# mikasenghaas/diloco-swarm

Measured on AMD Instinct MI355X. Metric: GB/s params reduced (device-resident), DiLoCo outer step @1/2/4/8 GPU, higher is better.
Workload: dtype f32; 1 GPU; DiLoCo outer step, t125 tree per rank, through the reference's calls (src/train.py:263-269) on get_outer_model's default (CPU) outer model, stepped on its HBM twin: one dl_delta_pack_sgd per step (delta + outer.grad + Nesterov SGD + copy to inner; no exchange at one replica, src/comm.py:118-119); tree=t125, placement=host (write_back lazy: HBM twin), params=124475904, tensors=148, wire=f32, buckets=2, exchange=none (one peer), parallelism=dp1

## Files before the change

### __graft_entry__.py

```python
import os
import subprocess
import sys

HERE = os.path.dirname(os.path.abspath(__file__))
PKG = os.path.join(HERE, "diloco-swarm_amd")
for _p in (PKG, HERE):
    if _p not in sys.path:
        sys.path.insert(0, _p)


def build() -> None:
    env = dict(os.environ)
    env.setdefault("PYTORCH_ROCM_ARCH", "gfx950")
    subprocess.run(["make", "-s", "-C", os.path.join(PKG, "csrc")], check=True, env=env)
    subprocess.run(["make", "-s", "-C", os.path.join(HERE, "oracle")], check=True, env=env)
    cabi = os.path.join(HERE, "tests", "cabi")
    subprocess.run(
        ["gcc", "-O2", "-std=c11", "-D__HIP_PLATFORM_AMD__", "-I/opt/rocm/include",
         os.path.join(cabi, "host_step.c"), "-o", os.path.join(cabi, "host_step"),
         "-L" + os.path.join(PKG, "lib"), "-ldiloco_hip", "-L" + os.path.join(HERE, "oracle"),
         "-loracle", "-L/opt/rocm/lib", "-lamdhip64",
         "-Wl,-rpath,$ORIGIN/../../diloco-swarm_amd/lib", "-Wl,-rpath,$ORIGIN/../../oracle",
         "-Wl,-rpath,/opt/rocm/lib"], check=True, env=env)
    import diloco_amd
    from diloco_amd import _lib

    _lib.load()


def smoke() -> None:
    import numpy as np
    import torch

    from diloco_amd import synth
    from diloco_amd.outer import OuterSync
    from diloco_amd.trees import get_tree
    from oracle import oracle

    dev = torch.device("cuda", 0)
    spec = get_tree("micro")
    shapes = [s for _, s in spec.params()]
    params = [t.view(s) for t, s in zip(synth.outer_tree_device(spec, dev), shapes)]
    eng = OuterSync(params, lr=0.7, momentum=0.9, nesterov=True, world_size=1, keep_wire=True)
    synth.inner_tree_device([p.view(-1) for p in params], 1, 0, out=[p.view(-1) for p in params])
    eng.step()
    torch.cuda.synchronize()
    got = np.concatenate([t.reshape(-1).cpu().numpy() for t in eng.unpacked(eng.theta)])
    inner = np.concatenate([p.reshape(-1).cpu().numpy() for p in params])
    wire = np.concatenate([t.reshape(-1).cpu().numpy() for t in eng.unpacked(eng.wire)])

    with np.load(os.path.join(HERE, "tests", "golden", "micro_n1.npz")) as g:
        ref_theta, ref_delta = g["theta_s1"], g["delta_s1_r0"]
    st = oracle.OuterState(synth.outer_tree(spec.numels(), spec.init_spec()))
    deltas, _ = st.step([synth.inner_tree(st.theta, 1, 0)])
    assert got.tobytes() == ref_theta.tobytes(), "HIP outer step != reference (micro, n=1)"
    assert got.tobytes() == np.concatenate(st.theta).tobytes(), "HIP outer step != oracle"
# ... 37 lines not shown
```

### diloco-swarm_amd/csrc/dl_abi.hip

```cpp
#include <cstdarg>
#include <cstdio>
#include <cstring>
#include <new>
#include <string>
#include <vector>

#include "dl_internal.h"

namespace {

thread_local std::string g_err;

int fail(int code, const char* fmt, ...) __attribute__((format(printf, 2, 3)));
int fail(int code, const char* fmt, ...) {
  char buf[512];
  va_list ap;
  va_start(ap, fmt);
  vsnprintf(buf, sizeof buf, fmt, ap);
  va_end(ap);
  g_err = buf;
  return code;
}

int hip_fail(hipError_t e, const char* where) {
// ... 39 lines not shown
}

struct dl_tree_s;
namespace {
int slot_begin(dl_tree_s* t, int32_t slot, hipStream_t s, const char* who);
int slot_end(dl_tree_s* t, int32_t slot, hipStream_t s, const char* who);
}

constexpr int kStageRing = 4;

struct dl_tree_s {
  int device = 0;
  int32_t nseg = 0;
  int64_t total = 0;
  std::vector<int64_t> numel, seg_off, bounds;
  std::vector<int32_t> bkt_chunk;
  std::vector<dl::Chunk> chunks;
  std::vector<int64_t> chunk_loff;
  dl::Chunk* d_chunks = nullptr;
  int64_t* d_loff = nullptr;
  void** d_caddr = nullptr;
  uint64_t* d_segptr = nullptr;
  uint64_t* h_stage = nullptr;
  hipEvent_t stage_ev[kStageRing] = {};
  bool stage_used[kStageRing] = {};
  int stage_next = 0;
  std::vector<uint8_t> bound;
  std::vector<uint8_t> slot_aligned;
  int32_t grid = 0;
  int32_t flags = DL_TUNE_AUTO;
  hipEvent_t slot_ev[DL_MAX_SLOTS] = {};
  hipStream_t slot_stream[DL_MAX_SLOTS] = {};
  bool slot_used[DL_MAX_SLOTS] = {};
};

namespace {
int slot_begin(dl_tree_s* t, int32_t slot, hipStream_t s, const char* who) {
  if (slot < 0) return DL_OK;
  if (t->slot_used[slot] && t->slot_stream[slot] != s)
    DL_HIP(hipStreamWaitEvent(s, t->slot_ev[slot], 0), who);
  return DL_OK;
}
int slot_end(dl_tree_s* t, int32_t slot, hipStream_t s, const char* who) {
  if (slot < 0) return DL_OK;
  DL_HIP(hipEventRecord(t->slot_ev[slot], s), who);
  t->slot_stream[slot] = s;
  t->slot_used[slot] = true;
  return DL_OK;
}
}

extern "C" {

DL_API const char* dl_last_error(void) { return g_err.c_str(); }
DL_API int dl_abi_version(void) { return DL_ABI_VERSION; }

DL_API int dl_plan_tables_ex(const int64_t* numel, int32_t n, int64_t cap_elems,
                             int32_t align_elems, int64_t bucket_align_elems, int64_t* seg_off,
                             int64_t* bkt_bounds, int32_t* n_bkt) {
  if (n < 0 || (n > 0 && !numel) || !seg_off || !bkt_bounds || !n_bkt)
    return fail(DL_E_ARG, "dl_plan_tables: null pointer or n < 0");
  if (align_elems <= 0) return fail(DL_E_ARG, "dl_plan_tables: align_elems must be > 0");
  if (bucket_align_elems <= 0 || bucket_align_elems % align_elems)
    return fail(DL_E_ARG, "dl_plan_tables: bucket_align %lld is not a positive multiple of %d",
                (long long)bucket_align_elems, align_elems);
  for (int32_t i = 0; i < n; ++i)
// ... 376 lines not shown
                                   float* wire, float* mom, float lr, float momentum,
                                   int32_t nesterov, int32_t first_step, dl_stream_t s) {
  dl::Launch L;
  DL_TRY(make_launch(t, b, s, &L, "dl_delta_pack_sgd_defer", kAutoUnpackSgd));
  DL_TRY(check_slot(t, inner_slot, "dl_delta_pack_sgd_defer"));
  DL_TRY(check_packed(outer, "dl_delta_pack_sgd_defer", "outer"));
  DL_TRY(check_packed(wire, "dl_delta_pack_sgd_defer", "wire"));
  dl::SgdArgs a;
  DL_TRY(sgd_args("dl_delta_pack_sgd_defer", mom, lr, momentum, nesterov, first_step, &a));
  DL_TRY(slot_begin(t, inner_slot, L.stream, "dl_delta_pack_sgd_defer"));
  hipError_t e = dl::launch_delta_pack_sgd_defer(L, inner_slot, outer, wire, mom, a);
  return e == hipSuccess ? slot_end(t, inner_slot, L.stream, "dl_delta_pack_sgd_defer") : hip_fail(e, "dl_delta_pack_sgd_defer");
}

DL_API int dl_delta_pack_sgd_resume(dl_tree_t t, int32_t b, int32_t inner_slot, float* outer,
                                    float* wire, float* mom, float pending_lr,
                                    float pending_momentum, int32_t pending_nesterov,
                                    int32_t pending_first_step, float lr, float momentum,
                                    int32_t nesterov, int32_t first_step, dl_stream_t s) {
  dl::Launch L;
  DL_TRY(make_launch(t, b, s, &L, "dl_delta_pack_sgd_resume", kAutoUnpackSgd));
  DL_TRY(check_slot(t, inner_slot, "dl_delta_pack_sgd_resume"));
  DL_TRY(check_packed(outer, "dl_delta_pack_sgd_resume", "outer"));
  DL_TRY(check_packed(wire, "dl_delta_pack_sgd_resume", "wire"));
  dl::SgdArgs p, a;
  DL_TRY(sgd_args("dl_delta_pack_sgd_resume", mom, pending_lr, pending_momentum, pending_nesterov,
                  pending_first_step, &p));
  DL_TRY(sgd_args("dl_delta_pack_sgd_resume", mom, lr, momentum, nesterov, first_step, &a));
  DL_TRY(slot_begin(t, inner_slot, L.stream, "dl_delta_pack_sgd_resume"));
  hipError_t e = dl::launch_delta_pack_sgd_resume(L, inner_slot, outer, wire, mom, p, a);
  return e == hipSuccess ? slot_end(t, inner_slot, L.stream, "dl_delta_pack_sgd_resume") : hip_fail(e, "dl_delta_pack_sgd_resume");
}

DL_API int dl_unpack_adamw(dl_tree_t t, int32_t b, const void* wire, int32_t wire_dtype,
                           int32_t divisor, float* outer, float* exp_avg, float* exp_avg_sq,
                           float decay, float w1, float beta2, float w2, float neg_step_size,
                           float bc2_sqrt, float eps, int32_t inner_slot, dl_stream_t s) {
  dl::Launch L;
  DL_TRY(make_launch(t, b, s, &L, "dl_unpack_adamw", kAutoUnpackSgd));
  DL_TRY(check_packed(wire, "dl_unpack_adamw", "wire"));
  DL_TRY(check_dtype(wire_dtype, "dl_unpack_adamw"));
  DL_TRY(check_packed(outer, "dl_unpack_adamw", "outer"));
  DL_TRY(check_packed(exp_avg, "dl_unpack_adamw", "exp_avg"));
  DL_TRY(check_packed(exp_avg_sq, "dl_unpack_adamw", "exp_avg_sq"));
  DL_TRY(check_slot(t, inner_slot, "dl_unpack_adamw", true));
  if (divisor < 1) return fail(DL_E_ARG, "dl_unpack_adamw: divisor %d", divisor);
  dl::AdamArgs a{decay, w1, beta2, w2, neg_step_size, bc2_sqrt, eps};
  DL_TRY(slot_begin(t, inner_slot, L.stream, "dl_unpack_adamw"));
  hipError_t e = dl::launch_unpack_adamw(L, wire, wire_dtype, divisor, outer, exp_avg, exp_avg_sq,
                                         a, inner_slot);
  return e == hipSuccess ? slot_end(t, inner_slot, L.stream, "dl_unpack_adamw") : hip_fail(e, "dl_unpack_adamw");
}

DL_API int dl_delta_pack_adamw(dl_tree_t t, int32_t b, int32_t inner_slot, float* outer,
                               void* wire, int32_t wire_dtype, float* exp_avg, float* exp_avg_sq,
                               float decay, float w1, float beta2, float w2, float neg_step_size,
                               float bc2_sqrt, float eps, dl_stream_t s) {
  dl::Launch L;
  DL_TRY(make_launch(t, b, s, &L, "dl_delta_pack_adamw", kAutoUnpackSgd));
  DL_TRY(check_slot(t, inner_slot, "dl_delta_pack_adamw"));
  DL_TRY(check_packed(outer, "dl_delta_pack_adamw", "outer"));
  DL_TRY(check_packed(wire, "dl_delta_pack_adamw", "wire"));
  DL_TRY(check_dtype(wire_dtype, "dl_delta_pack_adamw"));
  DL_TRY(check_packed(exp_avg, "dl_delta_pack_adamw", "exp_avg"));
  DL_TRY(check_packed(exp_avg_sq, "dl_delta_pack_adamw", "exp_avg_sq"));
  dl::AdamArgs a{decay, w1, beta2, w2, neg_step_size, bc2_sqrt, eps};
// ... 623 lines not shown
```

### diloco-swarm_amd/diloco_amd/_lib.py

```python
from __future__ import annotations

import ctypes
import os
import threading

_HERE = os.path.dirname(os.path.abspath(__file__))
LIB_PATH = os.environ.get(
    "DILOCO_HIP_LIB", os.path.join(os.path.dirname(_HERE), "lib", "libdiloco_hip.so")
)

ABI_VERSION = 8
ALIGN_ELEMS = 64
CHUNK_ELEMS = 4096
ALL_BUCKETS = -1
MAX_SLOTS = 4
Q8_SLOT_BYTES = 4160
FP4_SLOT_BYTES = 2176
IPC_HANDLE_BYTES = 64
DL_F32, DL_BF16, DL_F16, DL_U8 = 0, 1, 2, 3
TUNE_NT_LOADS, TUNE_NT_STORES, TUNE_WT_STORES, TUNE_PAIRS = 1, 2, 8, 16
TUNE_AUTO = -1
COPY_WIDE, COPY_READ, COPY_WRITE = 8, 16, 32


# ... 11 lines not shown
    "dl_plan_tables": (ctypes.c_int, [_pi64, _i32, _i64, _i32, _pi64, _pi64, _pi32]),
    "dl_plan_tables_ex": (ctypes.c_int, [_pi64, _i32, _i64, _i32, _i64, _pi64, _pi64, _pi32]),
    "dl_tree_create": (ctypes.c_int, [_pi64, _i32, _i64, ctypes.POINTER(_vp)]),
    "dl_tree_create_ex": (ctypes.c_int, [_pi64, _i32, _i64, _i64, ctypes.POINTER(_vp)]),
    "dl_tree_destroy": (ctypes.c_int, [_vp]),
    "dl_tree_query": (ctypes.c_int, [_vp, _pi64, _pi32, _pi32, _pi32]),
    "dl_tree_bucket_range": (ctypes.c_int, [_vp, _i32, _pi64, _pi64]),
    "dl_tree_seg_off": (ctypes.c_int, [_vp, _pi64]),
    "dl_tree_bucket_chunks": (ctypes.c_int, [_vp, _i32, _pi32, _pi32]),
    "dl_tree_bind": (ctypes.c_int, [_vp, _i32, _pu64, _i32, _vp]),
    "dl_tree_tune": (ctypes.c_int, [_vp, _i32, _i32]),
    "dl_tuning_build": (ctypes.c_int, []),
    "dl_delta_pack": (ctypes.c_int, [_vp, _i32, _i32, _vp, _vp, _i32, _vp]),
    "dl_unpack_avg": (ctypes.c_int, [_vp, _i32, _vp, _i32, _i32, _i32, _vp, _vp]),
    "dl_grad_sumsq": (ctypes.c_int, [_vp, _i32, _i32, _vp, _vp]),
    "dl_unpack_avg_sumsq": (ctypes.c_int, [_vp, _i32, _vp, _i32, _i32, _i32, _vp, _vp, _vp]),
    "dl_norm_finish": (ctypes.c_int, [_vp, _i32, _f32, _vp, _vp]),
    "dl_scale_by": (ctypes.c_int, [_vp, _i32, _i32, _vp, _vp]),
    "dl_unpack_sgd": (
        ctypes.c_int,
        [_vp, _i32, _vp, _i32, _i32, _vp, _vp, _f32, _f32, _i32, _i32, _i32, _vp],
    ),
    "dl_delta_sgd": (ctypes.c_int, [_vp, _i32, _i32, _vp, _vp, _f32, _f32, _i32, _i32, _vp]),
    "dl_delta_pack_sgd": (
        ctypes.c_int, [_vp, _i32, _i32, _vp, _vp, _i32, _vp, _f32, _f32, _i32, _i32, _vp],
    ),
    "dl_delta_pack_sgd_defer": (
        ctypes.c_int, [_vp, _i32, _i32, _vp, _vp, _vp, _f32, _f32, _i32, _i32, _vp],
    ),
    "dl_delta_pack_sgd_resume": (
        ctypes.c_int,
        [_vp, _i32, _i32, _vp, _vp, _vp, _f32, _f32, _i32, _i32, _f32, _f32, _i32, _i32, _vp],
    ),
    "dl_unpack_adamw": (
        ctypes.c_int,
        [_vp, _i32, _vp, _i32, _i32, _vp, _vp, _vp, _f32, _f32, _f32, _f32, _f32, _f32, _f32,
         _i32, _vp],
    ),
    "dl_delta_pack_adamw": (
        ctypes.c_int,
        [_vp, _i32, _i32, _vp, _vp, _i32, _vp, _vp, _f32, _f32, _f32, _f32, _f32, _f32, _f32,
         _vp],
    ),
    "dl_adamw_step": (
        ctypes.c_int,
        [_vp, _i32, _i32, _i32, _vp, _vp, _vp, _f32, _f32, _f32, _f32, _f32, _f32, _f32, _vp],
    ),
    "dl_pack_sgd_tiled": (
        ctypes.c_int,
        [_vp, _i32, _i32, _vp, _vp, _i32, _vp, _f32, _f32, _i32, _i32, _i32, _vp],
    ),
    "dl_shard_sgd": (
        ctypes.c_int, [_vp, _i32, _i32, _vp, _vp, _i64, _f32, _f32, _i32, _i32, _vp],
    ),
    "dl_shard_reduce_sgd": (
        ctypes.c_int, [_vp, _i32, _i32, _i64, _vp, _vp, _f32, _f32, _i32, _i32, _vp],
    ),
    "dl_shard_reduce_avg": (ctypes.c_int, [_vp, _i32, _i32, _i64, _vp, _vp]),
    "dl_shard_adamw": (
        ctypes.c_int,
        [_vp, _i32, _i32, _vp, _vp, _vp, _i64, _f32, _f32, _f32, _f32, _f32, _f32, _f32, _vp],
    ),
    "dl_shard_reduce_adamw": (
        ctypes.c_int,
        [_vp, _i32, _i32, _i64, _vp, _vp, _vp, _vp, _f32, _f32, _f32, _f32, _f32, _f32, _f32,
         _vp],
# ... 114 lines not shown
```

### diloco-swarm_amd/diloco_amd/kernels.py

```python
from __future__ import annotations

import ctypes

from typing import Optional, Sequence

import torch

from . import _lib
from .plan import DEFAULT_BUCKET_CAP_ELEMS, PackedTree

_DT = {torch.float32: _lib.DL_F32, torch.bfloat16: _lib.DL_BF16}


Q8_SLOT = _lib.Q8_SLOT_BYTES
FP4_SLOT = _lib.FP4_SLOT_BYTES


def wire_code(dtype: torch.dtype) -> int:
    try:
        return _DT[dtype]
    except KeyError:
        raise TypeError(f"unsupported packed dtype {dtype} (float32 or bfloat16)") from None


# ... 40 lines not shown
        _lib.call("dl_delta_pack", tree.handle, bucket, inner_slot, theta.data_ptr(),
                  wire.data_ptr(), wire_code(wire.dtype), _s(theta))

    def unpack_sgd(self, tree, bucket, wire, divisor, theta, mom, lr, momentum, nesterov,
                   first, inner_slot) -> None:
        _lib.call("dl_unpack_sgd", tree.handle, bucket, wire.data_ptr(), wire_code(wire.dtype),
                  int(divisor), theta.data_ptr(), _ptr(mom), float(lr), float(momentum),
                  int(nesterov), int(first), int(inner_slot), _s(theta))

    def delta_sgd(self, tree, bucket, inner_slot, theta, mom, lr, momentum, nesterov,
                  first) -> None:
        _lib.call("dl_delta_sgd", tree.handle, bucket, inner_slot, theta.data_ptr(), _ptr(mom),
                  float(lr), float(momentum), int(nesterov), int(first), _s(theta))

    def delta_pack_sgd(self, tree, bucket, inner_slot, theta, wire, mom, lr, momentum, nesterov,
                       first) -> None:
        _lib.call("dl_delta_pack_sgd", tree.handle, bucket, inner_slot, theta.data_ptr(),
                  wire.data_ptr(), wire_code(wire.dtype), _ptr(mom), float(lr), float(momentum),
                  int(nesterov), int(first), _s(theta))

    def delta_pack_sgd_defer(self, tree, bucket, inner_slot, theta, wire, mom, lr, momentum,
                             nesterov, first) -> None:
        _lib.call("dl_delta_pack_sgd_defer", tree.handle, bucket, inner_slot, theta.data_ptr(),
                  wire.data_ptr(), _ptr(mom), float(lr), float(momentum), int(nesterov),
                  int(first), _s(theta))

    def delta_pack_sgd_resume(self, tree, bucket, inner_slot, theta, wire, mom, pending, lr,
                              momentum, nesterov, first) -> None:
        p_lr, p_momentum, p_nesterov, p_first = pending
        _lib.call("dl_delta_pack_sgd_resume", tree.handle, bucket, inner_slot, theta.data_ptr(),
                  wire.data_ptr(), _ptr(mom), float(p_lr), float(p_momentum), int(p_nesterov),
                  int(p_first), float(lr), float(momentum), int(nesterov), int(first), _s(theta))

    def unpack_adamw(self, tree, bucket, wire, divisor, theta, exp_avg, exp_avg_sq, scalars,
                     inner_slot) -> None:
        _lib.call("dl_unpack_adamw", tree.handle, bucket, wire.data_ptr(), wire_code(wire.dtype),
                  int(divisor), theta.data_ptr(), exp_avg.data_ptr(), exp_avg_sq.data_ptr(),
                  *scalars, int(inner_slot), _s(theta))

    def delta_pack_adamw(self, tree, bucket, inner_slot, theta, wire, exp_avg, exp_avg_sq,
                         scalars) -> None:
        _lib.call("dl_delta_pack_adamw", tree.handle, bucket, inner_slot, theta.data_ptr(),
                  wire.data_ptr(), wire_code(wire.dtype), exp_avg.data_ptr(),
                  exp_avg_sq.data_ptr(), *scalars, _s(theta))

    def adamw_step(self, tree, bucket, param_slot, grad_slot, exp_avg, exp_avg_sq, scalars,
                   coef=None) -> None:
        _lib.call("dl_adamw_step", tree.handle, bucket, int(param_slot), int(grad_slot),
                  exp_avg.data_ptr(), exp_avg_sq.data_ptr(), _ptr(coef), *scalars, _s(exp_avg))

    def pack_sgd_tiled(self, tree, bucket, inner_slot, theta, wire, mom, lr, momentum,
                       nesterov, first, tile_chunks) -> None:
        _lib.call("dl_pack_sgd_tiled", tree.handle, bucket, inner_slot, theta.data_ptr(),
                  wire.data_ptr(), wire_code(wire.dtype), _ptr(mom), float(lr), float(momentum),
                  int(nesterov), int(first), int(tile_chunks), _s(theta))

    def shard_sgd(self, wire, divisor, theta, mom, lr, momentum, nesterov, first) -> None:
        _lib.call("dl_shard_sgd", wire.data_ptr(), wire_code(wire.dtype), int(divisor),
                  theta.data_ptr(), _ptr(mom), theta.numel(), float(lr), float(momentum),
                  int(nesterov), int(first), _s(theta))

    def shard_reduce_sgd(self, slices, n_slices, theta, mom, lr, momentum, nesterov,
                         first) -> None:
        _lib.call("dl_shard_reduce_sgd", slices.data_ptr(), wire_code(slices.dtype),
                  int(n_slices), theta.numel(), theta.data_ptr(), _ptr(mom), float(lr),
                  float(momentum), int(nesterov), int(first), _s(theta))
# ... 137 lines not shown
```

### diloco-swarm_amd/diloco_amd/mirror.py

```python
from __future__ import annotations

import warnings
import weakref
from collections import OrderedDict
from operator import is_
from typing import List, Optional, Sequence

import torch
import torch.distributed as dist

from . import _lib
from .kernels import default_kernels
from .outer import pipelined_buckets
from .plan import DEFAULT_BUCKET_CAP_ELEMS, SLOT_GRAD, SLOT_INNER, q8_slot_plan

ALL = _lib.ALL_BUCKETS
S_CHUNK = _lib.CHUNK_ELEMS


def _decode_fp4(sl: torch.Tensor) -> torch.Tensor:
    nch = sl.shape[0]
    G = S_CHUNK // 32
    e = sl[:, :G].to(torch.int32).repeat_interleave(32, dim=1)
    pay = sl[:, G:].to(torch.int32)
# ... 483 lines not shown
                 bucket_cap_elems: int = DEFAULT_BUCKET_CAP_ELEMS, fused: bool = False,
                 wire: str = "f32", exchange: str = "sharded", keep_params: bool = False,
                 error_feedback: bool = False):
        if wire not in OUTER_WIRES:
            raise ValueError(f"wire {wire!r}: one of {OUTER_WIRES}")
        if exchange not in OUTER_EXCHANGES:
            raise ValueError(f"exchange {exchange!r}: one of {OUTER_EXCHANGES}")
        if error_feedback and wire not in SLOT_WIRES:
            raise ValueError("error_feedback compensates the int8 / fp4 wire's quantiser; it "
                             "needs wire='int8' or wire='fp4'")
        self.error_feedback = bool(error_feedback)
        self._q8_res: Optional[torch.Tensor] = None
        self._q8_res_load: Optional[list] = None
        self.exchange = exchange
        self.params: List[torch.nn.Parameter] = module_params(outer_model)
        if not self.params:
            raise ValueError("outer model has no parameters")
        self.k = kernels or default_kernels()
        self.device = torch.device(device)
        for i, p in enumerate(self.params):
            if p.device != self.device and not (keep_params and p.device.type == "cpu"):
                raise ValueError(f"outer parameter {i} is on {p.device}, expected {self.device}")
            if p.dtype != torch.float32:
                raise TypeError(f"outer parameter {i}: {p.dtype}, the outer step is fp32")
        self.fused = fused
        self.numels = [p.numel() for p in self.params]
        self.tree = self.k.tree(self.numels, self.device, bucket_cap_elems, dp_bucket_align())
        self.offs = [int(o) for o in self.tree.seg_off[:-1]]
        z = dict(dtype=torch.float32, device=self.device)
        self._theta = torch.zeros(self.tree.total, **z)
        self.d_wire = torch.zeros(self.tree.total, **z)
        self._mom: Optional[torch.Tensor] = None
        self.defer_state = False
        self._pend: Optional[tuple] = None
        self.wire = wire
        self.d_wire16 = (torch.zeros(self.tree.total, dtype=torch.bfloat16, device=self.device)
                         if wire == "bf16" else None)
        self._sum16 = False
        self._works: Optional[list] = None
        self._views = {"theta": self._make_views(self._theta),
                       "wire": self._make_views(self.d_wire)}
        self._ptrs = {k: [v.data_ptr() for v in vs] for k, vs in self._views.items()}
        self.theta_touched = True
        self.grads_touched = True
        self._theta_ver = None
        self._shared_ver = fused and not keep_params
        host_grads = None
        if any(p.device != self.device for p in self.params):
            host_grads = [_GRAD.__get__(p) for p in self.params]
            for p in self.params:
                _GRAD.__set__(p, None)
            self._relay("theta", "data", force=True)
        self._relay_theta()
        if host_grads is not None:
            with torch.no_grad():
                for p, g, v in zip(self.params, host_grads, self._views["wire"]):
                    if g is not None:
                        v.copy_(g)
                        _GRAD.__set__(p, v)
        if fused:
            self._install_outer_parameters(outer_model, keep_params)
        self._delta = None
        self._div = 1
        self._target = None
        self._synced = None
        self._mom_src: Optional[List[torch.Tensor]] = None
        self._xmode: Optional[str] = None
        self._xgroup, self._xn, self._xrank = None, 1, 0
        self._mom_stale = False
        self._mom_shard = None
        self.d_recv: Optional[torch.Tensor] = None
        self._warned = False
        self.d_m1: Optional[torch.Tensor] = None
        self.d_m2: Optional[torch.Tensor] = None
        self._adam_src = None
        self._adam_stale = False
        self._adam_shard = None
        self.adamw_replicated = False

    def settle_state(self) -> None:
        pend, self._pend = self._pend, None
        if pend is not None:
            lr, momentum, nesterov, first = pend
            self.k.unpack_sgd(self.tree, ALL, self.d_wire, 1, self._theta,
                              self._mom if momentum != 0 else None, lr, momentum, nesterov,
                              first, -1)

    @property
    def d_theta(self) -> torch.Tensor:
        self.settle_state()
        return self._theta

    @property
    def d_mom(self) -> Optional[torch.Tensor]:
        self.settle_state()
        return self._mom

    @d_mom.setter
    def d_mom(self, value) -> None:
        self.settle_state()
        self._mom = value

    def _momentum_buffer(self, view: torch.Tensor, arena: str = "mom") -> "MomentumBuffer":
        t = view.as_subclass(MomentumBuffer)
        t.__dict__["_dl_mirror"] = weakref.ref(self)
        t.__dict__["_dl_arena"] = arena
        return t

    def __deepcopy__(self, memo):
        return None

    def __reduce_ex__(self, proto):
        return (_none, ())

    def _install_outer_parameters(self, model: torch.nn.Module, keep: bool = False) -> None:
        ref = weakref.ref(self)
        if keep:
            for p in self.params:
                p.__class__ = OuterParameter
# ... 610 lines not shown
                self._views["mom"] = [self._momentum_buffer(v) for v in plain]
                self._ptrs["mom"] = [v.data_ptr() for v in plain]
            bufs = self._views["mom"]
            src = self._mom_src
            if not (src is not None and len(host_bufs) == len(src)
                    and all(map(is_, host_bufs, src))):
                have = [b is not None for b in host_bufs]
                if any(have) and not all(have):
                    raise RuntimeError("momentum buffers exist for some outer parameters only")
                first = not any(have)
                if not first:
                    self.settle_state()
                    copied = 0
                    with torch.no_grad():
                        for b, v, e in zip(host_bufs, self._views["mom_plain"],
                                           self._ptrs["mom"]):
                            if _DATA_PTR(b) != e:
                                v.copy_(b)
                                copied += 1
                    if copied == len(host_bufs):
                        self._mom_stale = False
            else:
                first = False
            self._mom_src = bufs
        mom = self._mom if momentum != 0 else None
        sharded = delta is None and self._xmode in ("sharded", "a2a")
        q8 = delta is None and self._xmode == "q8"
        if (mom is not None and self._mom_stale and not first
                and not (sharded and self._mom_shard == (self._xgroup, self._xn, self._xrank))):
            self.gather_momentum()
        target, self._target = self._target, None
        write = target is not None
        if delta is not None and self.defer_state:
            pend, self._pend = self._pend, None
            if pend is None:
                self.k.delta_pack_sgd_defer(self.tree, ALL, SLOT_INNER, self._theta, self.d_wire,
                                            mom, lr, momentum, nesterov, first)
                self._pend = (lr, momentum, nesterov, first)
            else:
                self.k.delta_pack_sgd_resume(self.tree, ALL, SLOT_INNER, self._theta,
                                             self.d_wire, mom if pend[1] == 0 else self._mom,
                                             pend, lr, momentum, nesterov, first)
            self._mom_stale = False
        elif delta is not None:
            self.k.delta_pack_sgd(self.tree, ALL, SLOT_INNER, self.d_theta, self.d_wire, mom,
                                  lr, momentum, nesterov, first)
            self._mom_stale = False
        elif sharded:
            self._sharded_sgd(mom, lr, momentum, nesterov, first, target)
        elif q8:
            self._mom_stale = False
            self._q8_sgd(mom, lr, momentum, nesterov, first, target)
        else:
            self._mom_stale = False
            if write:
                self.k.bind(self.tree, SLOT_INNER, target[0], self.device, key=tuple(target[1]))
            wire = self.d_wire16 if self._sum16 else self.d_wire
            slot = SLOT_INNER if write else -1
            works, self._works = self._works, None
            if works is None:
                self.k.unpack_sgd(self.tree, ALL, wire, self._div, self.d_theta, mom, lr,
                                  momentum, nesterov, first, slot)
            else:
                for b, w in enumerate(works):
                    w.wait()
                    self.k.unpack_sgd(self.tree, b, wire, self._div, self.d_theta, mom, lr,
                                      momentum, nesterov, first, slot)
        self._synced = (target + (tver,)) if write else None
        return bufs

    def adamw_ready(self) -> bool:
# ... 487 lines not shown
```

### diloco-swarm_amd/diloco_amd/outer.py

```python
from __future__ import annotations

from typing import Callable, List, Optional, Sequence

import torch
import torch.distributed as dist

from . import _lib
from .kernels import Q8_SLOT, default_kernels
from .plan import DEFAULT_BUCKET_CAP_ELEMS, SLOT_INNER, q8_slot_plan

ALL = _lib.ALL_BUCKETS
DEFAULT_TILE_CHUNKS = 8192


def pipelined_buckets(n_buckets: int, pack: Callable[[int], None],
                      reduce: Callable[[int], object], unpack: Callable[[int], None]) -> None:
    works = [None] * n_buckets
    for b in range(n_buckets):
        pack(b)
        works[b] = reduce(b)
        if b >= 1:
            works[b - 1].wait()
            unpack(b - 1)
    if n_buckets:
# ... 66 lines not shown
            rank = dist.get_rank(group) if dist.is_initialized() and self.world_size > 1 else 0
        self.rank = int(rank)
        if wire_dtype not in (torch.float32, torch.bfloat16, torch.int8):
            raise ValueError(f"wire dtype {wire_dtype}: float32, bfloat16 or int8")
        self.q8 = wire_dtype == torch.int8
        self.error_feedback = bool(error_feedback)
        if self.error_feedback and not self.q8:
            raise ValueError("error_feedback compensates the int8 wire's quantiser; it needs "
                             "wire_dtype=torch.int8")
        shard_given = shard
        if shard is None:
            shard = self.world_size > 1 and wire_dtype == torch.float32
        if shard and self.q8:
            raise ValueError("the int8 wire has its own exchange; shard=True needs f32/bf16")
        if exchange not in ("rccl", "a2a", "xgmi", "xgmi_inner"):
            raise ValueError(f"exchange {exchange!r}: 'rccl', 'a2a', 'xgmi' or 'xgmi_inner'")
        self.a2a = exchange == "a2a"
        if self.a2a:
            if self.q8:
                raise ValueError("exchange='a2a' exchanges the f32 or bf16 wire")
            if shard_given is False:
                raise ValueError("exchange='a2a' is a sharded step (shard=False contradicts it)")
            shard = True
        self.xgmi = exchange in ("xgmi", "xgmi_inner")
        self.xgmi_inner = exchange == "xgmi_inner"
        if self.xgmi and wire_dtype != torch.float32:
            raise ValueError(f"exchange={exchange!r} sends the fp32 wire")
        self.sharded = bool(shard) and not self.xgmi
        balign = _lib.ALIGN_ELEMS * (self.world_size if (self.sharded or self.xgmi) else 1)
        self.tree = self.k.tree([p.numel() for p in self.params], self.device, bucket_cap_elems,
                                balign)
        self.k.bind(self.tree, SLOT_INNER, self.params, self.device)
        z = dict(device=self.device)
        self.theta = torch.zeros(self.tree.total, dtype=torch.float32, **z)
        self.mom = (torch.zeros(self.tree.total, dtype=torch.float32, **z)
                    if self.momentum != 0 and not (self.sharded or self.xgmi) else None)
        if self.q8:
            n = self.world_size
            plan, base, _owned, mmax = q8_slot_plan(self.tree.bucket_chunks, n)
            self.q8_plan = [(nch, m, at) for nch, m, at, _rat in plan]
            self.wire = None
            self.q_slots = torch.zeros(base * Q8_SLOT, dtype=torch.uint8, **z)
            self.q_recv = torch.zeros(n * mmax * Q8_SLOT, dtype=torch.uint8, **z)
            self.q_red = torch.zeros(mmax * Q8_SLOT, dtype=torch.uint8, **z)
            self.q_residual = self.q_residual_red = None
            if self.error_feedback:
                self.q_residual = torch.zeros(self.tree.total, dtype=torch.float32, **z)
                if n > 1:
                    self.q_residual_red = [
                        torch.zeros(m * _lib.CHUNK_ELEMS, dtype=torch.float32, **z)
                        for _nch, m, _base in self.q8_plan]
        elif self.xgmi_inner:
            self.wire = None
        else:
            self.wire = torch.zeros(self.tree.total, dtype=wire_dtype, **z)
        self.k.gather(self.tree, ALL, SLOT_INNER, self.theta)
        if self.sharded:
            n, r = self.world_size, self.rank
            self.shard_off, off = [], 0
            for lo, hi in self.tree.bucket_ranges:
                assert (hi - lo) % n == 0
                self.shard_off.append(off)
                off += (hi - lo) // n
            self.shard_total = off
            self.th_shard = torch.empty(off, dtype=torch.float32, **z)
            for b in range(self.tree.n_buckets):
                self.th_shard_view(b).copy_(self.theta_shard_of(b))
            self.g_shard = None if self.a2a else torch.zeros(off, dtype=wire_dtype, **z)
            self.mom_shard = (torch.zeros(off, dtype=torch.float32, **z)
                              if self.momentum != 0 else None)
            self.a2a_recv: Optional[List[torch.Tensor]] = None
        if self.xgmi:
            from .xgmi import PeerMap

            n = self.world_size
            self.x_len = self.tree.total // n
            self.x_lo = self.rank * self.x_len
            self.mom_x = (torch.zeros(self.x_len, dtype=torch.float32, **z)
                          if self.momentum != 0 else None)
            self._flag = torch.zeros(1, dtype=torch.float32, **z)
            if self.xgmi_inner:
                self._relay_inner()
            src = self.inner_arena if self.xgmi_inner else self.wire
            self.peers = PeerMap({"src": src, "theta": self.theta},
                                 group if n > 1 else None, self.device)
            if not self.peers.ok:
                raise RuntimeError(f"exchange='xgmi' unavailable: {self.peers.reason}")
        self.steps_done = 0
        self._step_bound = False
        if side_stream is None:
            side_stream = not (self.world_size == 1 and self.fuse_single and not self.q8
                               and not self.xgmi and not self.sharded)
        self.stream = (torch.cuda.Stream(self.device)
                       if side_stream and self.device.type == "cuda" else None)

    def _relay_inner(self) -> None:
        z = dict(dtype=torch.float32, device=self.device)
        self.inner_arena = torch.zeros(self.tree.total, **z)
        with torch.no_grad():
            for i, o in enumerate(self._objs):
                lo = int(self.tree.seg_off[i])
                v = self.inner_arena[lo:lo + o.numel()].view(o.shape)
                v.copy_(o.data if isinstance(o, torch.nn.Parameter) else o)
                o.data = v
        self.params = [o.data if isinstance(o, torch.nn.Parameter) else o for o in self._objs]
        self._arena_ptrs = [o.data_ptr() for o in self._objs]
        self.k.bind(self.tree, SLOT_INNER, self.params, self.device)

    def _bind_inner(self) -> None:
        if not self._step_bound:
            self.k.bind(self.tree, SLOT_INNER, self.params, self.device)

    def pseudo_gradient(self, bucket: int = ALL) -> None:
        if self.xgmi_inner:
            raise RuntimeError("exchange='xgmi_inner' has no wire: the exchange kernel forms "
                               "the pseudo-gradient; use step()")
        self._bind_inner()
        if self.q8:
            self._delta_q8(bucket, self.q8_region(bucket))
        else:
            self.k.delta_pack(self.tree, bucket, SLOT_INNER, self.theta, self.wire)

    def _delta_q8(self, bucket: int, slots: torch.Tensor) -> None:
        if self.error_feedback:
            self.k.delta_q8_ef(self.tree, bucket, SLOT_INNER, self.theta, self.q_residual, slots)
        else:
            self.k.delta_q8(self.tree, bucket, SLOT_INNER, self.theta, slots)
# ... 142 lines not shown
            self._step(pipeline)
            return
        cur = torch.cuda.current_stream(self.device)
        if cur == self.stream:
            self._step(pipeline)
            return
        self.stream.wait_stream(cur)
        with torch.cuda.stream(self.stream):
            self._step(pipeline)
        cur.wait_stream(self.stream)

    def _step(self, pipeline: Optional[bool]) -> None:
        if pipeline is None:
            pipeline = self.world_size > 1
        if not self.xgmi_inner:
            self.k.bind(self.tree, SLOT_INNER, self.params, self.device)
        self._step_bound = True
        try:
            self._step_body(pipeline)
        finally:
            self._step_bound = False
        self.steps_done += 1

    def _step_body(self, pipeline: bool) -> None:
        if self.q8:
            self._step_q8(pipeline)
        elif self.xgmi:
            self._step_xgmi()
        elif self.sharded:
            self._step_sharded()
        elif pipeline:
            pipelined_buckets(self.tree.n_buckets, self.pseudo_gradient,
                              lambda b: self.all_reduce(b, async_op=True), self.apply)
        elif self.fuse_single and self.keep_wire:
            self.k.delta_pack_sgd(self.tree, ALL, SLOT_INNER, self.theta, self.wire, self.mom,
                                  self.lr, self.momentum, self.nesterov, self.steps_done == 0)
        elif self.fuse_single:
            self.k.delta_sgd(self.tree, ALL, SLOT_INNER, self.theta, self.mom, self.lr,
                             self.momentum, self.nesterov, self.steps_done == 0)
        elif self.tile_chunks:
            self.k.pack_sgd_tiled(self.tree, ALL, SLOT_INNER, self.theta, self.wire, self.mom,
                                  self.lr, self.momentum, self.nesterov, self.steps_done == 0,
                                  self.tile_chunks)
        else:
            self.pseudo_gradient(ALL)
            self.apply(ALL)

    def _step_sharded(self) -> None:
        nb = self.tree.n_buckets
        rs, ag = [None] * nb, [None] * nb
        self.pseudo_gradient(0)
        rs[0] = self.reduce_scatter(0)
        for b in range(nb):
            if b + 1 < nb:
                self.pseudo_gradient(b + 1)
                rs[b + 1] = self.reduce_scatter(b + 1)
            rs[b].wait()
            self.shard_apply(b)
            ag[b] = self.all_gather(b)
            if b >= 1:
                ag[b - 1].wait()
                self.write_inner(b - 1)
        ag[nb - 1].wait()
        self.write_inner(nb - 1)

    def _barrier(self) -> None:
# ... 71 lines not shown
                    dst.copy_(src.view(dst.shape))
                if self.xgmi:
                    self.mom_x.copy_(full[self.x_lo:self.x_lo + self.x_len])
                elif self.sharded:
                    for b in range(self.tree.n_buckets):
                        lo, _ = self.tree.bucket_ranges[b]
                        s = self._shard_len(b)
                        self._shard(self.mom_shard, b).copy_(
                            full[lo + self.rank * s:lo + (self.rank + 1) * s])
                else:
                    self.mom.copy_(full)
            if self.sharded:
                for b in range(self.tree.n_buckets):
                    self.th_shard_view(b).copy_(self.theta_shard_of(b))
        self.steps_done = int(state["steps"])
        if write_inner:
            self.k.bind(self.tree, SLOT_INNER, self.params, self.device)
            self.k.scatter(self.tree, ALL, self.theta, SLOT_INNER)

    def unpacked(self, packed: torch.Tensor) -> List[torch.Tensor]:
        out = []
        for i, p in enumerate(self.params):
            lo = int(self.tree.seg_off[i])
            out.append(packed[lo:lo + p.numel()].view(p.shape))
        return out

    def close(self) -> None:
        if getattr(self, "peers", None) is not None:
            if self.world_size > 1:
                torch.cuda.synchronize(self.device)
                dist.barrier(group=self.group)
            self.peers.close()
            self.peers = None
        self.tree.close()
```

### include/diloco_hip.h

```cpp
#ifndef DILOCO_HIP_H
#define DILOCO_HIP_H

#include <stdint.h>

#ifdef __cplusplus
extern "C" {
#endif

#define DL_API __attribute__((visibility("default")))

#define DL_ABI_VERSION 8
#define DL_ALIGN_ELEMS 64
#define DL_CHUNK_ELEMS 4096
#define DL_ALL_BUCKETS (-1)
#define DL_MAX_SLOTS 4
#define DL_Q8_SLOT_BYTES 4160
#define DL_FP4_SLOT_BYTES 2176

#define DL_F32 0
#define DL_BF16 1
#define DL_F16 2
#define DL_U8 3

#define DL_OK 0
// ... 47 lines not shown
DL_API int dl_unpack_avg_sumsq(dl_tree_t tree, int32_t bucket, const void* wire,
                               int32_t wire_dtype, int32_t divisor, int32_t dst_slot,
                               float* dst_packed, double* partials, dl_stream_t stream);
DL_API int dl_norm_finish(const double* partials, int32_t n_partials, float max_norm,
                          float* out2, dl_stream_t stream);
DL_API int dl_scale_by(dl_tree_t tree, int32_t bucket, int32_t slot, const float* coef,
                       dl_stream_t stream);

DL_API int dl_unpack_sgd(dl_tree_t tree, int32_t bucket, const void* wire, int32_t wire_dtype,
                         int32_t divisor, float* outer_packed, float* mom_packed, float lr,
                         float momentum, int32_t nesterov, int32_t first_step,
                         int32_t inner_slot, dl_stream_t stream);

DL_API int dl_delta_sgd(dl_tree_t tree, int32_t bucket, int32_t inner_slot, float* outer_packed,
                        float* mom_packed, float lr, float momentum, int32_t nesterov,
                        int32_t first_step, dl_stream_t stream);

DL_API int dl_delta_pack_sgd(dl_tree_t tree, int32_t bucket, int32_t inner_slot,
                             float* outer_packed, void* wire, int32_t wire_dtype,
                             float* mom_packed, float lr, float momentum, int32_t nesterov,
                             int32_t first_step, dl_stream_t stream);

DL_API int dl_delta_pack_sgd_defer(dl_tree_t tree, int32_t bucket, int32_t inner_slot,
                                   float* outer_packed, float* wire, float* mom_packed, float lr,
                                   float momentum, int32_t nesterov, int32_t first_step,
                                   dl_stream_t stream);

DL_API int dl_delta_pack_sgd_resume(dl_tree_t tree, int32_t bucket, int32_t inner_slot,
                                    float* outer_packed, float* wire, float* mom_packed,
                                    float pending_lr, float pending_momentum,
                                    int32_t pending_nesterov, int32_t pending_first_step,
                                    float lr, float momentum, int32_t nesterov,
                                    int32_t first_step, dl_stream_t stream);

DL_API int dl_unpack_adamw(dl_tree_t tree, int32_t bucket, const void* wire, int32_t wire_dtype,
                           int32_t divisor, float* outer_packed, float* exp_avg_packed,
                           float* exp_avg_sq_packed, float decay, float w1, float beta2, float w2,
                           float neg_step_size, float bc2_sqrt, float eps, int32_t inner_slot,
                           dl_stream_t stream);

DL_API int dl_delta_pack_adamw(dl_tree_t tree, int32_t bucket, int32_t inner_slot,
                               float* outer_packed, void* wire, int32_t wire_dtype,
                               float* exp_avg_packed, float* exp_avg_sq_packed, float decay,
                               float w1, float beta2, float w2, float neg_step_size,
                               float bc2_sqrt, float eps, dl_stream_t stream);

DL_API int dl_adamw_step(dl_tree_t tree, int32_t bucket, int32_t param_slot, int32_t grad_slot,
                         float* exp_avg_packed, float* exp_avg_sq_packed, const float* coef,
                         float decay, float w1, float beta2, float w2, float neg_step_size,
                         float bc2_sqrt, float eps, dl_stream_t stream);

DL_API int dl_pack_sgd_tiled(dl_tree_t tree, int32_t bucket, int32_t inner_slot,
                             float* outer_packed, void* wire, int32_t wire_dtype,
                             float* mom_packed, float lr, float momentum, int32_t nesterov,
                             int32_t first_step, int32_t tile_chunks, dl_stream_t stream);

DL_API int dl_gather(dl_tree_t tree, int32_t bucket, int32_t src_slot, void* packed,
                     int32_t dtype, dl_stream_t stream);

DL_API int dl_scatter(dl_tree_t tree, int32_t bucket, const float* packed, int32_t dst_slot,
                      dl_stream_t stream);

DL_API int dl_shard_sgd(const void* wire, int32_t wire_dtype, int32_t divisor, float* outer,
                        float* mom, int64_t n, float lr, float momentum, int32_t nesterov,
                        int32_t first_step, dl_stream_t stream);

// ... 119 lines not shown
```

Baseline: 967.0 GB/s.

## Move deferred outer-SGD state bookkeeping into the library with settle-on-read

```diff
diff --git a/__graft_entry__.py b/__graft_entry__.py
--- a/__graft_entry__.py
+++ b/__graft_entry__.py
@@ -15,13 +15,14 @@
     subprocess.run(["make", "-s", "-C", os.path.join(PKG, "csrc")], check=True, env=env)
     subprocess.run(["make", "-s", "-C", os.path.join(HERE, "oracle")], check=True, env=env)
     cabi = os.path.join(HERE, "tests", "cabi")
-    subprocess.run(
-        ["gcc", "-O2", "-std=c11", "-D__HIP_PLATFORM_AMD__", "-I/opt/rocm/include",
-         os.path.join(cabi, "host_step.c"), "-o", os.path.join(cabi, "host_step"),
-         "-L" + os.path.join(PKG, "lib"), "-ldiloco_hip", "-L" + os.path.join(HERE, "oracle"),
-         "-loracle", "-L/opt/rocm/lib", "-lamdhip64",
-         "-Wl,-rpath,$ORIGIN/../../diloco-swarm_amd/lib", "-Wl,-rpath,$ORIGIN/../../oracle",
-         "-Wl,-rpath,/opt/rocm/lib"], check=True, env=env)
+    for host in ("host_step", "host_cycle"):
+        subprocess.run(
+            ["gcc", "-O2", "-std=c11", "-D__HIP_PLATFORM_AMD__", "-I/opt/rocm/include",
+             os.path.join(cabi, host + ".c"), "-o", os.path.join(cabi, host),
+             "-L" + os.path.join(PKG, "lib"), "-ldiloco_hip", "-L" + os.path.join(HERE, "oracle"),
+             "-loracle", "-L/opt/rocm/lib", "-lamdhip64",
+             "-Wl,-rpath,$ORIGIN/../../diloco-swarm_amd/lib", "-Wl,-rpath,$ORIGIN/../../oracle",
+             "-Wl,-rpath,/opt/rocm/lib"], check=True, env=env)
     import diloco_amd
     from diloco_amd import _lib
 
diff --git a/diloco-swarm_amd/csrc/dl_abi.hip b/diloco-swarm_amd/csrc/dl_abi.hip
--- a/diloco-swarm_amd/csrc/dl_abi.hip
+++ b/diloco-swarm_amd/csrc/dl_abi.hip
@@ -95,6 +95,14 @@
   hipEvent_t slot_ev[DL_MAX_SLOTS] = {};
   hipStream_t slot_stream[DL_MAX_SLOTS] = {};
   bool slot_used[DL_MAX_SLOTS] = {};
+  struct PendingSgd {
+    bool on = false;
+    float* outer = nullptr;
+    float* wire = nullptr;
+    float* mom = nullptr;
+    float lr = 0.f, momentum = 0.f;
+    int32_t nesterov = 0, first_step = 0;
+  } pend;
 };
 
 namespace {
@@ -537,6 +545,63 @@
   return e == hipSuccess ? slot_end(t, inner_slot, L.stream, "dl_delta_pack_sgd_resume") : hip_fail(e, "dl_delta_pack_sgd_resume");
 }
 
+DL_API int dl_outer_sgd_step(dl_tree_t t, int32_t inner_slot, float* outer, float* wire,
+                             float* mom, float lr, float momentum, int32_t nesterov,
+                             int32_t first_step, int32_t defer_ok, dl_stream_t s) {
+  const char* who = "dl_outer_sgd_step";
+  dl::Launch L;
+  DL_TRY(make_launch(t, DL_ALL_BUCKETS, s, &L, who, kAutoUnpackSgd));
+  DL_TRY(check_slot(t, inner_slot, who));
+  DL_TRY(check_packed(outer, who, "outer"));
+  DL_TRY(check_packed(wire, who, "wire"));
+  dl::SgdArgs a;
+  DL_TRY(sgd_args(who, mom, lr, momentum, nesterov, first_step, &a));
+  dl_tree_s::PendingSgd& p = t->pend;
+  if (p.on && (outer != p.outer || wire != p.wire || (mom && p.mom && mom != p.mom)))
+    return fail(DL_E_ARG,
+                "%s: a step is pending in other buffers (outer %p, wire %p, momentum %p); "
+                "dl_outer_sgd_settle first", who, (void*)p.outer, (void*)p.wire, (void*)p.mom);
+  DL_TRY(slot_begin(t, inner_slot, L.stream, who));
+  hipError_t e;
+  if (p.on) {
+    dl::SgdArgs pa;
+    DL_TRY(sgd_args(who, p.mom, p.lr, p.momentum, p.nesterov, p.first_step, &pa));
+    e = dl::launch_delta_pack_sgd_resume(L, inner_slot, outer, wire, p.mom ? p.mom : mom, pa, a);
+    if (e == hipSuccess) p = dl_tree_s::PendingSgd{};
+  } else if (defer_ok) {
+    e = dl::launch_delta_pack_sgd_defer(L, inner_slot, outer, wire, mom, a);
+    if (e == hipSuccess) {
+      p.on = true;
+      p.outer = outer, p.wire = wire, p.mom = momentum != 0.f ? mom : nullptr;
+      p.lr = lr, p.momentum = momentum;
+      p.nesterov = nesterov ? 1 : 0, p.first_step = first_step ? 1 : 0;
+    }
+  } else {
+    e = dl::launch_delta_pack_sgd(L, inner_slot, outer, wire, DL_F32, mom, a);
+  }
+  return e == hipSuccess ? slot_end(t, inner_slot, L.stream, who) : hip_fail(e, who);
+}
+
+DL_API int dl_outer_sgd_settle(dl_tree_t t, dl_stream_t s) {
+  const char* who = "dl_outer_sgd_settle";
+  dl::Launch L;
+  DL_TRY(make_launch(t, DL_ALL_BUCKETS, s, &L, who, kAutoUnpackSgd));
+  dl_tree_s::PendingSgd& p = t->pend;
+  if (!p.on) return DL_OK;
+  dl::SgdArgs a;
+  DL_TRY(sgd_args(who, p.mom, p.lr, p.momentum, p.nesterov, p.first_step, &a));
+  hipError_t e = dl::launch_unpack_sgd(L, p.wire, DL_F32, 1, p.outer, p.mom, a, -1);
+  if (e != hipSuccess) return hip_fail(e, who);
+  p = dl_tree_s::PendingSgd{};
+  return DL_OK;
+}
+
+DL_API int dl_outer_sgd_pending(dl_tree_t t, int32_t* out) {
+  if (!t || !out) return fail(DL_E_ARG, "dl_outer_sgd_pending: null argument");
+  *out = t->pend.on ? 1 : 0;
+  return DL_OK;
+}
+
 DL_API int dl_unpack_adamw(dl_tree_t t, int32_t b, const void* wire, int32_t wire_dtype,
                            int32_t divisor, float* outer, float* exp_avg, float* exp_avg_sq,
                            float decay, float w1, float beta2, float w2, float neg_step_size,
diff --git a/diloco-swarm_amd/diloco_amd/_lib.py b/diloco-swarm_amd/diloco_amd/_lib.py
--- a/diloco-swarm_amd/diloco_amd/_lib.py
+++ b/diloco-swarm_amd/diloco_amd/_lib.py
@@ -67,6 +67,11 @@
         ctypes.c_int,
         [_vp, _i32, _i32, _vp, _vp, _vp, _f32, _f32, _i32, _i32, _f32, _f32, _i32, _i32, _vp],
     ),
+    "dl_outer_sgd_step": (
+        ctypes.c_int, [_vp, _i32, _vp, _vp, _vp, _f32, _f32, _i32, _i32, _i32, _vp],
+    ),
+    "dl_outer_sgd_settle": (ctypes.c_int, [_vp, _vp]),
+    "dl_outer_sgd_pending": (ctypes.c_int, [_vp, _pi32]),
     "dl_unpack_adamw": (
         ctypes.c_int,
         [_vp, _i32, _vp, _i32, _i32, _vp, _vp, _vp, _f32, _f32, _f32, _f32, _f32, _f32, _f32,
diff --git a/diloco-swarm_amd/diloco_amd/kernels.py b/diloco-swarm_amd/diloco_amd/kernels.py
--- a/diloco-swarm_amd/diloco_amd/kernels.py
+++ b/diloco-swarm_amd/diloco_amd/kernels.py
@@ -96,6 +96,21 @@
                   wire.data_ptr(), _ptr(mom), float(p_lr), float(p_momentum), int(p_nesterov),
                   int(p_first), float(lr), float(momentum), int(nesterov), int(first), _s(theta))
 
+    def outer_sgd_step(self, tree, inner_slot, theta, wire, mom, lr, momentum, nesterov, first,
+                       defer_ok) -> None:
+        _lib.call("dl_outer_sgd_step", tree.handle, inner_slot, theta.data_ptr(),
+                  wire.data_ptr(), _ptr(mom), float(lr), float(momentum), int(nesterov),
+                  int(first), int(defer_ok), _s(theta))
+
+    def outer_sgd_settle(self, tree, device) -> None:
+        _lib.call("dl_outer_sgd_settle", tree.handle,
+                  torch.cuda.current_stream(device).cuda_stream)
+
+    def outer_sgd_pending(self, tree) -> bool:
+        out = ctypes.c_int32(0)
+        _lib.call("dl_outer_sgd_pending", tree.handle, ctypes.byref(out))
+        return bool(out.value)
+
     def unpack_adamw(self, tree, bucket, wire, divisor, theta, exp_avg, exp_avg_sq, scalars,
                      inner_slot) -> None:
         _lib.call("dl_unpack_adamw", tree.handle, bucket, wire.data_ptr(), wire_code(wire.dtype),
diff --git a/diloco-swarm_amd/diloco_amd/mirror.py b/diloco-swarm_amd/diloco_amd/mirror.py
--- a/diloco-swarm_amd/diloco_amd/mirror.py
+++ b/diloco-swarm_amd/diloco_amd/mirror.py
@@ -539,7 +539,8 @@
         self.d_wire = torch.zeros(self.tree.total, **z)
         self._mom: Optional[torch.Tensor] = None
         self.defer_state = False
-        self._pend: Optional[tuple] = None
+        self._lib_cycle = hasattr(self.k, "outer_sgd_step")
+        self._pend_host: Optional[tuple] = None
         self.wire = wire
         self.d_wire16 = (torch.zeros(self.tree.total, dtype=torch.bfloat16, device=self.device)
                          if wire == "bf16" else None)
@@ -586,12 +587,26 @@
         self.adamw_replicated = False
 
     def settle_state(self) -> None:
-        pend, self._pend = self._pend, None
+        if self._lib_cycle:
+            if self._lib_pending():
+                self.k.outer_sgd_settle(self.tree, self.device)
+            return
+        pend, self._pend_host = self._pend_host, None
         if pend is not None:
             lr, momentum, nesterov, first = pend
             self.k.unpack_sgd(self.tree, ALL, self.d_wire, 1, self._theta,
                               self._mom if momentum != 0 else None, lr, momentum, nesterov,
                               first, -1)
+
+    def _lib_pending(self) -> bool:
+        return (self.defer_state and getattr(self.tree, "_h", True) is not None
+                and self.k.outer_sgd_pending(self.tree))
+
+    @property
+    def _pend(self):
+        if self._lib_cycle:
+            return (True,) if self._lib_pending() else None
+        return self._pend_host
 
     @property
     def d_theta(self) -> torch.Tensor:
@@ -1268,11 +1283,14 @@
         target, self._target = self._target, None
         write = target is not None
         if delta is not None and self.defer_state:
-            pend, self._pend = self._pend, None
-            if pend is None:
+            pend, self._pend_host = self._pend_host, None
+            if self._lib_cycle:
+                self.k.outer_sgd_step(self.tree, SLOT_INNER, self._theta, self.d_wire, mom, lr,
+                                      momentum, nesterov, first, True)
+            elif pend is None:
                 self.k.delta_pack_sgd_defer(self.tree, ALL, SLOT_INNER, self._theta, self.d_wire,
                                             mom, lr, momentum, nesterov, first)
-                self._pend = (lr, momentum, nesterov, first)
+                self._pend_host = (lr, momentum, nesterov, first)
             else:
                 self.k.delta_pack_sgd_resume(self.tree, ALL, SLOT_INNER, self._theta,
                                              self.d_wire, mom if pend[1] == 0 else self._mom,
diff --git a/diloco-swarm_amd/diloco_amd/outer.py b/diloco-swarm_amd/diloco_amd/outer.py
--- a/diloco-swarm_amd/diloco_amd/outer.py
+++ b/diloco-swarm_amd/diloco_amd/outer.py
@@ -122,9 +122,14 @@
                                 balign)
         self.k.bind(self.tree, SLOT_INNER, self.params, self.device)
         z = dict(device=self.device)
-        self.theta = torch.zeros(self.tree.total, dtype=torch.float32, **z)
-        self.mom = (torch.zeros(self.tree.total, dtype=torch.float32, **z)
-                    if self.momentum != 0 and not (self.sharded or self.xgmi) else None)
+        self._theta = torch.zeros(self.tree.total, dtype=torch.float32, **z)
+        self._mom = (torch.zeros(self.tree.total, dtype=torch.float32, **z)
+                     if self.momentum != 0 and not (self.sharded or self.xgmi) else None)
+        from .utils import env_flag
+
+        self._cycle = (self.keep_wire and self.fuse_single and wire_dtype == torch.float32
+                       and hasattr(self.k, "outer_sgd_step"))
+        self.defer_state = self._cycle and env_flag("DILOCO_OUTER_DEFER_STATE", True)
         if self.q8:
             n = self.world_size
             plan, base, _owned, mmax = q8_slot_plan(self.tree.bucket_chunks, n)
@@ -183,6 +188,29 @@
                                and not self.xgmi and not self.sharded)
         self.stream = (torch.cuda.Stream(self.device)
                        if side_stream and self.device.type == "cuda" else None)
+
+    def settle_state(self) -> None:
+        if self.pending():
+            self.k.outer_sgd_settle(self.tree, self.device)
+
+    def pending(self) -> bool:
+        return (self.defer_state and getattr(self.tree, "_h", True) is not None
+                and self.k.outer_sgd_pending(self.tree))
+
+    @property
+    def theta(self) -> torch.Tensor:
+        self.settle_state()
+        return self._theta
+
+    @property
+    def mom(self) -> Optional[torch.Tensor]:
+        self.settle_state()
+        return self._mom
+
+    @mom.setter
+    def mom(self, value) -> None:
+        self.settle_state()
+        self._mom = value
 
     def _relay_inner(self) -> None:
         z = dict(dtype=torch.float32, device=self.device)
@@ -391,6 +419,10 @@
         elif pipeline:
             pipelined_buckets(self.tree.n_buckets, self.pseudo_gradient,
                               lambda b: self.all_reduce(b, async_op=True), self.apply)
+        elif self._cycle:
+            self.k.outer_sgd_step(self.tree, SLOT_INNER, self._theta, self.wire, self._mom,
+                                  self.lr, self.momentum, self.nesterov, self.steps_done == 0,
+                                  self.defer_state)
         elif self.fuse_single and self.keep_wire:
             self.k.delta_pack_sgd(self.tree, ALL, SLOT_INNER, self.theta, self.wire, self.mom,
                                   self.lr, self.momentum, self.nesterov, self.steps_done == 0)
@@ -528,4 +560,5 @@
                 dist.barrier(group=self.group)
             self.peers.close()
             self.peers = None
+        self.settle_state()
         self.tree.close()
diff --git a/include/diloco_hip.h b/include/diloco_hip.h
--- a/include/diloco_hip.h
+++ b/include/diloco_hip.h
@@ -103,6 +103,13 @@
                                     int32_t pending_nesterov, int32_t pending_first_step,
                                     float lr, float momentum, int32_t nesterov,
                                     int32_t first_step, dl_stream_t stream);
+
+DL_API int dl_outer_sgd_step(dl_tree_t tree, int32_t inner_slot, float* outer_packed,
+                             float* wire, float* mom_packed, float lr, float momentum,
+                             int32_t nesterov, int32_t first_step, int32_t defer_ok,
+                             dl_stream_t stream);
+DL_API int dl_outer_sgd_settle(dl_tree_t tree, dl_stream_t stream);
+DL_API int dl_outer_sgd_pending(dl_tree_t tree, int32_t* pending);
 
 DL_API int dl_unpack_adamw(dl_tree_t tree, int32_t bucket, const void* wire, int32_t wire_dtype,
                            int32_t divisor, float* outer_packed, float* exp_avg_packed,
```

After: 963.9 GB/s. About the same (-0.3%).
